# Mesoptier/ray-marching

Hardware: AMD Instinct MI355X
Metric: Mpixels/s at 1920x1080, 256-step march, 32-node SDF (higher is better)
Workload: dtype f32; 1 GPU; 1920x1080, g32 (31 commands / 111 words), 256 max steps, 16 rays/px, RGBA32F out; camera=still, kernel=0, specialized_kernel=True, jit_from_disk_cache=True, frames_in_flight=4

## Files before the change

### ray-marching_amd/csrc/rm_jit.h

```cpp
#pragma once
#include <algorithm>
#include <atomic>
#include <chrono>
#include <condition_variable>
#include <cstdio>
#include <cstdlib>
#include <cstring>
#include <dlfcn.h>
#include <sys/stat.h>
#include <unistd.h>
#include <map>
#include <memory>
#include <mutex>
#include <string>
#include <thread>
#include <vector>

#include "rm_device.h"
#include "rm_units.h"

namespace rmjit {

#include "generated/rm_jit_sources.inc"

// ... 531 lines not shown
            const int w = nv++;
            char an[16], am[16], bn[16], bm[16];
            std::snprintf(an, sizeof an, "v%d", a); std::snprintf(am, sizeof am, "m%d", a);
            std::snprintf(bn, sizeof bn, "v%d", b); std::snprintf(bm, sizeof bm, "m%d", b);
            if (!combine(w, an, am, bn, bm)) return false;
            stack.push_back(w);
            continue;
        }
        const char* fn = kind == RM_KIND_SPHERE ? "sdf_sphere_t<FAST>" : kind == RM_KIND_BOX ? "sdf_box_t<FAST>"
                       : kind == RM_KIND_CYLINDER ? "sdf_cylinder_t<FAST>" : nullptr;
        const int c = pos.back();
        const int leaf = nv++;
        if (fn) std::snprintf(line, sizeof line, "    const float v%d = %s(x%d, y%d, z%d, mp[%u].p, tiny);\n", leaf, fn, c, c, c, r);
        else if (kind == RM_KIND_PLANE)
            std::snprintf(line, sizeof line, "    const float v%d = ((x%d * mp[%u].p[0] + y%d * mp[%u].p[1]) + z%d * mp[%u].p[2]) + mp[%u].p[3];\n", leaf, c, r, c, r, c, r, r);
        else return false;
        s += line;
        if (fn) s += "    guard_fence(tiny);\n";
        if (++leaves % 2 == 0) s += "    __builtin_amdgcn_sched_barrier(0);\n";
        if (mode == RM_MODE_PUSH) {
            std::snprintf(line, sizeof line, "    const uint32_t m%d = 0u;\n", leaf);
            s += line;
            stack.push_back(leaf);
        } else {
            if (stack.empty() || mode == RM_MODE_SMOOTH) return false;
            const int a = stack.back(); stack.pop_back();
            const int w = nv++;
            char an[16], am[16], bn[16];
            std::snprintf(an, sizeof an, "v%d", a); std::snprintf(am, sizeof am, "m%d", a); std::snprintf(bn, sizeof bn, "v%d", leaf);
            if (!combine(w, an, am, bn, "0u")) return false;
            stack.push_back(w);
        }
    }
    if (stack.empty()) return false;
    std::snprintf(line, sizeof line, "    return m%d;\n}\n}  // namespace rmk\n", stack.back());
    s += line;
    *out = std::move(s);
    return true;
}

inline const char* kernel_name() { return "rm_render_v5_spec"; }

inline bool structure_allows_bound_walk(const std::vector<RmRecord>& rec) {
    bool smooth = false;
    int spilled = 0, depth = 0;
    for (const RmRecord& r : rec) {
        const uint32_t kind = RM_OP_KIND(r.op);
        if (kind == RM_KIND_XFORM || kind == RM_KIND_MATERIAL) return false;
        smooth = smooth || RM_OP_MODE(r.op) == RM_MODE_SMOOTH || RM_OP_MODE(r.op) == RM_MODE_INTER || kind == RM_KIND_PLANE;
        if (kind == RM_KIND_POP) spilled--;
        else if (r.op & RM_OP_SPILL) spilled++;
        depth = spilled > depth ? spilled : depth;
    }
    return smooth && depth <= 1;
}

inline bool generate_source(const std::vector<RmRecord>& rec, const std::vector<RmRecord>& mrec, int wpt, int prune_kind, std::string* out,
                            bool* walk_generated = nullptr, bool* taps4_generated = nullptr, std::string* capped_out = nullptr) {
    const bool materials = !mrec.empty();
    const bool with_stats = (prune_kind & KERNEL_WITH_STATS) != 0;
    const bool range_proved = range_variant(prune_kind, materials);
    prune_kind &= PRUNE_KIND_MASK;
    std::string body, taps, walk, unit_walk;
    if (!generate_scene_code(rec, prune_kind, 1, &body, &unit_walk)) return false;
    const bool walk_spec = materials && mrec.size() <= kMaxRecords && generate_material_walk(mrec, &walk);
    if (walk_generated) *walk_generated = walk_spec;
    const bool taps4 = generate_scene_code(rec, prune_kind, 4, &taps);
    if (taps4_generated) *taps4_generated = taps4;
    std::string s;
    s += "typedef unsigned char rm_rtc_u8;\ntypedef unsigned short rm_rtc_u16;\ntypedef unsigned int rm_rtc_u32;\n"
         "typedef unsigned long long rm_rtc_u64;\ntypedef int rm_rtc_i32;\ntypedef long long rm_rtc_i64;\n"
         "#define uint8_t rm_rtc_u8\n#define uint16_t rm_rtc_u16\n#define uint32_t rm_rtc_u32\n#define uint64_t rm_rtc_u64\n"
         "#define int32_t rm_rtc_i32\n#define int64_t rm_rtc_i64\n";
    s += "#define RM_JIT_TU 1\n";
    if (prune_kind == PRUNE_LATTICE) s += "#define RM_JIT_PRUNE_ON 1\n";
    if (prune_kind == PRUNE_BLEND) s += "#define RM_JIT_BLEND_PRUNE 1\n";
    if (taps4) s += "#define RM_JIT_TAPS4 1\n";
    if (walk_spec) s += "#define RM_JIT_MATERIAL_WALK 1\n";
    if (structure_allows_bound_walk(rec)) s += "#define RM_JIT_BOUND_WALK 1\n";
    if (!with_stats) s += "#define RM_NO_WAVE_STATS 1\n";
    if (range_proved) s += "#define RM_JIT_RANGE_PROOF 1\n";
    if (!unit_walk.empty()) s += "#define RM_JIT_UNIT_WALK 1\n";
    if (prune_kind && jit_knob("RM_JIT_PRUNE_STATS", 0) == 5) s += "#define RM_JIT_WALK_COUNTER 1\n";
    s += "#include \"rm_kernel_v5.h\"\n";
    s += body;
    s += unit_walk;
    if (taps4) s += taps;
    if (walk_spec) s += walk;
    char line[512];
    int waves = prune_kind == PRUNE_BLEND ? 6 : 0;
    bool chain = !materials && taps4 && prune_kind != PRUNE_BLEND && !rec.empty();
    for (size_t i = 1; chain && i < rec.size(); i++) {
        const uint32_t kind = RM_OP_KIND(rec[i].op), mode = RM_OP_MODE(rec[i].op);
        chain = (kind == RM_KIND_SPHERE || kind == RM_KIND_BOX || kind == RM_KIND_CYLINDER || kind == RM_KIND_PLANE) && mode != RM_MODE_PUSH;
    }
    if (chain) waves = 7;
    const bool probe = capped_out && waves == 0 && prune_kind == PRUNE_LATTICE && !materials && jit_knob("RM_JIT_PROBE_CAP", 1) != 0;
    auto kernel_text = [&](int w) {
        std::string k;
        if (w > 0) {
            std::snprintf(line, sizeof line, "__attribute__((amdgpu_waves_per_eu(%d, %d)))\n", w, w);
            k += line;
        }
        std::snprintf(line, sizeof line,
                      "extern \"C\" __global__ __launch_bounds__(%d) void %s(RmLaunch L, rmk::V5Work work, uint32_t n_tiles, "
                      "uint32_t refill_min) {\n    rmk::rm_render_v5_body<rmk::ProgLds, true, %d, false, true, %s>(L, work, n_tiles, refill_min);\n}\n",
                      64 * wpt, kernel_name(), wpt, materials ? "true" : "false");
        k += line;
        return k;
    };
    if (capped_out) *capped_out = probe ? s + kernel_text(6) : std::string();
    s += kernel_text(waves);
    *out = std::move(s);
    return true;
}

struct CacheHeader {
    char magic[8];
    uint64_t bytes;
    uint64_t checksum;
    uint64_t reserved;
};
inline uint64_t fnv1a(const char* p, size_t n, uint64_t h = 1469598103934665603ull) {
    for (size_t i = 0; i < n; i++) { h ^= (unsigned char)p[i]; h *= 1099511628211ull; }
    return h;
}
inline const char* const* compile_options(int* n) {
    static const char* const opts[] = {"--offload-arch=gfx950", "-O3", "-std=c++17", "-ffp-contract=off", "-fno-slp-vectorize"};
    *n = (int)(sizeof opts / sizeof *opts);
    return opts;
}
inline std::string cache_dir() {
    if (const char* env = std::getenv("RM_JIT_CACHE_DIR")) return (env[0] == 0 || std::strcmp(env, "off") == 0) ? std::string() : std::string(env);
    Dl_info info;
    std::memset(&info, 0, sizeof info);
    if (!dladdr(reinterpret_cast<void*>(&cache_dir), &info) || !info.dli_fname) return std::string();
    std::string lib(info.dli_fname);
    const size_t slash = lib.rfind('/');
    if (slash == std::string::npos) return std::string();
    return lib.substr(0, slash) + "/jit_cache";
}
inline std::string cache_path(const std::string& src) {
    const std::string dir_s = cache_dir();
    const char* dir = dir_s.empty() ? nullptr : dir_s.c_str();
    Rtc& rtc = Rtc::get();
    if (!dir || !rtc.ok()) return std::string();
    uint64_t h = fnv1a(src.data(), src.size());
    for (int i = 0; i < kNumHeaders; i++) h = fnv1a(kHeaderSources[i], std::strlen(kHeaderSources[i]), h);
    int n_opts = 0;
    const char* const* opts = compile_options(&n_opts);
    for (int i = 0; i < n_opts; i++) h = fnv1a(opts[i], std::strlen(opts[i]) + 1, h);
    h = fnv1a(rtc.identity.data(), rtc.identity.size(), h);
    char name[64];
    std::snprintf(name, sizeof name, "/rm_%016llx.co", (unsigned long long)h);
    return std::string(dir) + name;
}

inline bool compile(const std::string& src, std::vector<char>* code, std::string* log, double* ms, bool* from_cache = nullptr) {
    Rtc& rtc = Rtc::get();
    if (from_cache) *from_cache = false;
    if (!rtc.ok()) { *log = rtc.error; return false; }
    const auto t0 = std::chrono::steady_clock::now();
    const std::string cache_file = cache_path(src);
    if (!cache_file.empty()) {
        if (FILE* f = std::fopen(cache_file.c_str(), "rb")) {
            CacheHeader hd;
// ... 258 lines not shown
```

### ray-marching_amd/csrc/rm_kernel_v5.h

```cpp
#pragma once
#include "rm_interp.h"
#include "rm_lds_layout.h"

namespace rmk {

typedef const __attribute__((address_space(3))) float* LdsF;
RM_DEV LdsF lds_vector_base(const void* generic_lds_ptr) {
    const uint32_t s = (uint32_t)(__SIZE_TYPE__)(const __attribute__((address_space(3))) void*)generic_lds_ptr;
    uint32_t v;
    asm("v_mov_b32 %0, %1" : "=v"(v) : "s"(s));
    return (LdsF)(__SIZE_TYPE__)v;
}
template <bool FAST>
RM_DEV float map_scene_spec(LdsF lp, float qx, float qy, float qz, unsigned long long need, unsigned long long live, SqrtGuard& tiny, uint32_t& n_eval);
#ifdef RM_JIT_UNIT_WALK
template <bool FAST>
RM_DEV float map_scene_walk(LdsF lp, float qx, float qy, float qz, unsigned long long need, unsigned long long live, SqrtGuard& tiny, uint32_t& n_eval);
#define RM_MAP_SCENE_STEP map_scene_walk
#else
#define RM_MAP_SCENE_STEP map_scene_spec
#endif
#ifdef RM_JIT_MATERIAL_WALK
template <bool FAST>
RM_DEV uint32_t map_scene_material_spec(const RmRecord* __restrict__ mp, float qx, float qy, float qz, SqrtGuard& tiny);
// ... 451 lines not shown
                const float slope = CONE ? nd - nn * (rho * 1.00001f) : nd;
                const float away = 1.0e-5f * nn;
                b = slope >= away ? v0 - (1.0e-5f * (__builtin_fabsf(v0) + __builtin_fabsf(p[3])) + nn * (4.0f * lower)) : -inf;
                bounded = false;
            } else if (kind == RM_KIND_SPHERE) {
                const float cx = __builtin_fmaf(my, dz, -(mz * dy)), cy = __builtin_fmaf(mz, dx, -(mx * dz)), cz = __builtin_fmaf(mx, dy, -(my * dx));
                const float perp2 = __builtin_fmaf(cz, cz, __builtin_fmaf(cy, cy, cx * cx));
                reach = fmax_(p[3], 0.0f);
                const float along = __builtin_fmaf(mz, dz, __builtin_fmaf(my, dy, mx * dx));
                const float dist = __builtin_amdgcn_sqrtf(along > 0.0f ? perp2 : mm);
                b = dist * (1.0f - 1.0e-5f) - p[3];
            } else {
                const bool cyl = kind == RM_KIND_CYLINDER;
                const float hx = fmax_(p[3], 0.0f), hy = fmax_(p[4], 0.0f), hz = cyl ? hx : fmax_(p[5], 0.0f);
                reach = (hx + hy) + hz;
                const float x1 = (mx - hx) * ix, x2 = (mx + hx) * ix, y1 = (my - hy) * iy, y2 = (my + hy) * iy;
                const float z1 = (mz - hz) * iz, z2 = (mz + hz) * iz;
                const float nx = fmin_(x1, x2), fx = fmax_(x1, x2), ny = fmin_(y1, y2), fy = fmax_(y1, y2);
                const float nz = fmin_(z1, z2), fz = fmax_(z1, z2);
                const float d0 = fmax_((nx - fy) * wxy, (ny - fx) * wxy);
                const float d1 = fmax_((nx - fz) * wxz, (nz - fx) * wxz);
                const float d2 = fmax_((ny - fz) * wyz, (nz - fy) * wyz);
                const float d3 = fmax_(-fx * ax, fmax_(-fy * ay, -fz * az));
                const float delta = fmax_(fmax_(d0, d1), fmax_(d2, d3));
                b = delta * (1.0f - 1.0e-5f);
            }
            if (CONE && bounded) b = b - (rho * 1.00001f) * ((__builtin_amdgcn_sqrtf(mm) * 1.00001f + reach) + fmax_(b, 0.0f));
            b = fmax_(b - (lower + 1.0e-5f * __builtin_fabsf(b)), -3.0e38f);
            if (op & RM_OP_SPILL) spilled = acc;
            a = acc;
        }
        if (mode == RM_MODE_PUSH) acc = b;
        else if (mode == RM_MODE_UNION) acc = fmin_(a, b);
        else if (mode == RM_MODE_SUB) acc = a;
        else if (mode == RM_MODE_INTER) acc = fmax_(a, b);
        else {
            const float kk = p[0];
            float v = fmin_(a, b);
            if (kk > 0.0f) {
                const float h = fmax_(kk - __builtin_fabsf(a - b), 0.0f) * __builtin_amdgcn_rcpf(kk);
                v = v - ((h * h) * kk) * 0.25f;
                v = v - (1.0e-6f * (__builtin_fabsf(v) + kk));
            }
            acc = fmax_(v, -3.0e38f);
        }
    }
    return acc;
}
template <bool CONE, class LoadRecord>
RM_DEV bool ray_misses_by_bounds_v5(const LoadRecord& load, uint32_t n_rec, const V4& ro, float dx, float dy, float dz, float min_dist,
                                    float scale, float rho = 0.0f) {
    const float acc = ray_bound_v5<CONE>(load, n_rec, ro, dx, dy, dz, scale, rho);
    const float margin = fmax_(min_dist, 0.0f) * 1.01f + 1.0e-4f * scale;
    return acc > margin;
}

struct V5Work {
    const uint32_t* order;
    uint32_t* counters;
    uint32_t* measured;
    const uint32_t* masks;
};

RM_DEV float select_by_mask(float a, float b, unsigned long long m) {
    float r;
    asm("v_cndmask_b32_e64 %0, %1, %2, %3" : "=v"(r) : "v"(a), "v"(b), "s"(m));
    return r;
}
RM_DEV uint32_t select_by_mask(uint32_t a, uint32_t b, unsigned long long m) {
    uint32_t r;
    asm("v_cndmask_b32_e64 %0, %1, %2, %3" : "=v"(r) : "v"(a), "v"(b), "s"(m));
    return r;
}
RM_DEV bool lane_of(unsigned long long m, uint32_t lane) {
    uint32_t r;
    asm("v_cndmask_b32_e64 %0, 0, 1, %1" : "=v"(r) : "s"(m));
    (void)lane;
    return r != 0u;
}

struct TrueTag { static constexpr bool value = true; };
struct FalseTag { static constexpr bool value = false; };

template <class Prog, bool PROG_IN_LDS, int WPT, bool EXT, bool SPEC, bool MAT = false, int LOOP = 0>
RM_DEV void rm_render_v5_body(const RmLaunch& L, const V5Work& work, uint32_t n_tiles, uint32_t refill_min) {
    extern __shared__ __attribute__((aligned(16))) uint32_t smem[];
    const uint32_t tid = threadIdx.x;
    const uint32_t lane = tid & 63u, wave = tid >> 6;
    typedef rml::MarchWaveLds WL;
    float* res = reinterpret_cast<float*>(smem);
    uint32_t* wbase = smem + V5_POOL + wave * L.wave_dwords;
    uint32_t* rq_rid = wbase + WL::rq_rid / 4u;
    float* rq_d = reinterpret_cast<float*>(wbase + WL::rq_d / 4u);
    uint32_t* sq_rid = wbase + WL::sq_rid / 4u;
    float* sq_v = reinterpret_cast<float*>(wbase + WL::sq_v / 4u);
    uint32_t* hq_rid = wbase + WL::hq_rid / 4u;
    float* hq_v = reinterpret_cast<float*>(wbase + WL::hq_v / 4u);
    float* wxy = reinterpret_cast<float*>(wbase + WL::wxy / 4u);
    float* tn = reinterpret_cast<float*>(wbase + WL::tn / 4u);
    uint32_t* after = smem + V5_POOL + WPT * L.wave_dwords;
    float* spill = reinterpret_cast<float*>(after) + wave * (L.spill_depth * 64u) + lane;
    float4* t_cone = reinterpret_cast<float4*>(after + WPT * L.spill_depth * 64u);
    float4* t_slab = t_cone + L.n_cone;
    uint32_t* lprog = reinterpret_cast<uint32_t*>(t_slab + 3u * L.n_slab);
    uint32_t* s_next = lprog + (PROG_IN_LDS ? (L.n_rec + L.n_grp + L.n_tree) * 8u : 0u);
    uint32_t* s_tile = s_next + 1;
    uint32_t* s_veto = s_next + 2;
    float* s_off = reinterpret_cast<float*>(s_next + rml::kMarchCtlBytes / 4u);
    uint8_t* rmat = reinterpret_cast<uint8_t*>(s_next) + rml::kMarchCtlBytes + rml::kMarchOffBytes;
    uint32_t* s_mask = reinterpret_cast<uint32_t*>(rmat + (MAT && L.n_mrec != 0u ? V5_POOL : 0u));
    const bool tagged = MAT && L.n_mrec != 0u;
    constexpr uint32_t TAP_IDLE = MAT ? 5u : 4u;
    const CullTables cullt{t_cone, t_slab, s_veto, L.n_cone, L.n_slab};

    rm_uniforms u = L.u;
    if (L.frames) u = L.frames[blockIdx.z];
    const uint32_t tiles_x = (L.W + 7u) / 8u;
    const uint32_t* order = work.order + (size_t)blockIdx.z * n_tiles;
    uint32_t* counters = work.counters + 4u * blockIdx.z;
    const uint32_t n_active = counters[0];

    const V4 ro = matvec(u.inv_view, 0.0f, 0.0f, 0.0f, 1.0f);
    const float prune_scale = L.scene_scale + ((__builtin_fabsf(ro.x) + __builtin_fabsf(ro.y)) + __builtin_fabsf(ro.z));
    const float thr_c0 = step_thr_c0(prune_scale, ro.x, ro.y, ro.z);
    const float eps = 0.0001f;
    if (PROG_IN_LDS) {
        const uint32_t* src = reinterpret_cast<const uint32_t*>(L.prog);
        for (uint32_t k = tid; k < L.n_rec * 8u; k += 64u * WPT) lprog[SPEC ? ((k & ~7u) | ((k + 7u) & 7u)) : k] = src[k];
        stage_units(lprog + 8u * L.n_rec, L.prog + L.n_rec, L.n_grp, tid, 64u * WPT);
        if constexpr (!SPEC) stage_tree(lprog + 8u * (L.n_rec + L.n_grp), L.prog + L.n_rec + L.n_grp, L.n_tree, tid, 64u * WPT);
    }
    if (tid == 0u) *s_veto = 0u;
    if (tid < 16u) sample_offset(u, tid >> 2, tid & 3u, s_off[2u * tid], s_off[2u * tid + 1u]);
    __syncthreads();
    if (L.flags & 1u)
        for (uint32_t k = tid; k < L.n_rec; k += 64u * WPT) cull_build_v5(L.prog[k], ro, L.min_dist, L.smooth_slack, t_cone, t_slab, s_veto, L.bounds);

    Prog prog;
    if constexpr (PROG_IN_LDS) prog.base = lprog;
    else prog.base = L.prog;

    auto load_record = [&](uint32_t i, uint32_t& op, float (&p)[7]) {
        if constexpr (PROG_IN_LDS) {
            const uint32_t* r = lprog + 8u * i;
            op = r[SPEC ? 7u : 0u];
#pragma unroll
            for (int k = 0; k < 7; k++) p[k] = __uint_as_float(r[(SPEC ? 0u : 1u) + (uint32_t)k]);
        } else {
            prog.load(i, op, p);
        }
    };
    const float bound_scale = prune_scale + L.smooth_slack;
    const LdsF lprog_v = lds_vector_base(lprog);
    uint32_t n_eval = 0u;
    const uint32_t* lunits = lprog + 8u * L.n_rec;
    auto units_needed = [&](float x, float y, float z, float thr, float extra_margin, bool is_live, unsigned long long live_mask) -> unsigned long long {
        if constexpr (SPEC) {
#if defined(RM_JIT_PRUNE_ON)
            return wave_cull_lattice(lunits, L.n_grp, x, y, z, thr, is_live, live_mask);
#elif defined(RM_JIT_BLEND_PRUNE)
            return wave_cull_blend(lunits, L.n_grp, L.unit_kmax, x, y, z, extra_margin, prune_scale, is_live, live_mask);
#else
            return ~0ull;
#endif
        } else if constexpr (LOOP == 2 || LOOP == 4) {
            return wave_cull_lattice(lunits, L.n_grp, x, y, z, thr, is_live, live_mask);
        } else if constexpr (LOOP == 1 || LOOP == 3) {
            return ~0ull;
        } else if constexpr (PROG_IN_LDS) {
            if ((L.flags & 8u) == 0u) return ~0ull;
            if (L.unit_mode == RM_UNITS_LATTICE) return wave_cull_lattice(lunits, L.n_grp, x, y, z, thr, is_live, live_mask);
            return wave_cull_blend(lunits, L.n_grp, L.unit_kmax, x, y, z, extra_margin, prune_scale, is_live, live_mask);
        } else {
            return ~0ull;
        }
    };
    auto eval_scene = [&](float x, float y, float z, float thr, bool is_live, unsigned long long live_mask) -> float {
        float qx[1] = {x}, qy[1] = {y}, qz[1] = {z}, v[1];
        SqrtGuard tiny;
        if constexpr (SPEC) {
            const unsigned long long need = units_needed(x, y, z, thr, 0.0f, is_live, live_mask);
            v[0] = RM_MAP_SCENE_STEP<true>(lprog_v, x, y, z, need, live_mask, tiny, n_eval);
            if (tiny.any_bad()) {
                asm volatile("");
                uint32_t again = 0u;
                v[0] = RM_MAP_SCENE_STEP<false>(lprog_v, x, y, z, need, live_mask, tiny, again);
            }
        } else if (LOOP == 1 || LOOP == 2 || (LOOP == 0 && (L.flags & 4u))) {
            const unsigned long long need = units_needed(x, y, z, thr, 0.0f, is_live, live_mask);
            const bool masked = LOOP == 0 ? (PROG_IN_LDS && (L.flags & 8u) != 0u) : LOOP == 2;
#ifdef RM_INTERP_STATS
            n_eval += (uint32_t)__builtin_popcountll(masked ? need : (L.n_rec >= 64u ? ~0ull : (1ull << L.n_rec) - 1ull));
#endif
            v[0] = map_scene_chain<true>(prog, L.n_rec, x, y, z, need, masked, tiny);
            if (tiny.any_bad()) v[0] = map_scene_chain<false>(prog, L.n_rec, x, y, z, need, masked, tiny);
        } else if (LOOP == 3 || LOOP == 4 || (LOOP == 0 && !EXT)) {
            const bool masked = LOOP == 0 ? (PROG_IN_LDS && (L.flags & 8u) != 0u) : LOOP == 4;
            if (masked) {
                const unsigned long long need = units_needed(x, y, z, thr, 0.0f, is_live, live_mask);
                const TreeKeep k = tree_keep(lunits + 8u * L.n_grp, L.n_rec, need);
#ifdef RM_INTERP_STATS
                n_eval += (uint32_t)(__builtin_popcountll(k.keep0) + __builtin_popcountll(k.keep1));
#endif
                v[0] = map_scene_tree_masked<true>(prog, spill, x, y, z, k.keep0, k.keep1, k.push0, k.push1, tiny);
                if (tiny.any_bad()) v[0] = map_scene_tree_masked<false>(prog, spill, x, y, z, k.keep0, k.keep1, k.push0, k.push1, tiny);
            } else {
                v[0] = map_scene_tree<true>(prog, L.n_rec, spill, x, y, z, tiny);
                if (tiny.any_bad()) v[0] = map_scene_tree<false>(prog, L.n_rec, spill, x, y, z, tiny);
            }
        } else if (PROG_IN_LDS && (L.flags & 8u)) {
            const unsigned long long need = units_needed(x, y, z, thr, 0.0f, is_live, live_mask);
            const uint32_t* ranges = lunits + 7u * L.n_grp;
            v[0] = map_scene_units<true, EXT>(prog, ranges, spill, x, y, z, need, tiny, L.value_spill_depth);
            if (tiny.any_bad())
                v[0] = map_scene_units<false, EXT>(prog, ranges, spill, x, y, z, need, tiny, L.value_spill_depth);
        } else {
            map_scene_multi<1, true, Prog, EXT>(prog, L.n_rec, spill, L.max_dist, qx, qy, qz, v, tiny, L.value_spill_depth);
            if (tiny.any_bad()) map_scene_multi<1, false, Prog, EXT>(prog, L.n_rec, spill, L.max_dist, qx, qy, qz, v, tiny, L.value_spill_depth);
        }
        return v[0];
    };

    enum : uint32_t { START_MARCH = 0u, START_HIT = 1u, START_DONE = 2u };
    const float f0 = __uint_as_float(__builtin_amdgcn_readfirstlane(counters[2]));
    uint32_t start = START_DONE;
    if (L.max_iter != 0u)
        start = f0 < L.min_dist ? START_HIT : (f0 > L.max_dist || L.max_iter <= 1u) ? START_DONE : START_MARCH;
    const float inf_f = __uint_as_float(0x7F800000u);
#if defined(RM_JIT_PRUNE_ON)
    constexpr bool ANCHOR = SPEC;
#elif defined(RM_PRUNE_PLUMBING)
    constexpr bool ANCHOR = !SPEC && (LOOP == 2 || LOOP == 4);
#else
    constexpr bool ANCHOR = false;
#endif
    float anc_x = 0.0f, anc_y = 0.0f, anc_z = 0.0f, anc_t = inf_f;
    unsigned long long anc_due = 0ull;

    const unsigned long long t_start = L.stats ? __builtin_amdgcn_s_memrealtime() : 0ull;
    uint32_t n_iter = 0u, n_live = 0u, n_prod = 0u, n_tiles_done = 0u;

  for (;;) {
    if (tid == 0u) {
        *s_tile = atomicAdd(&counters[1], 1u);
        *s_next = 0u;
        s_next[3] = 0u;
    }
    __syncthreads();
    const uint32_t slot = *s_tile;
    if (slot >= n_active) break;
    const uint32_t tile = order[slot];
    const uint32_t tile_x = tile % tiles_x, tile_y = tile / tiles_x;
    n_tiles_done++;
    const unsigned long long tile_t0 = work.measured ? __builtin_amdgcn_s_memrealtime() : 0ull;

    if (lane < 16u) {
        const uint32_t k = lane & 7u, tx = tile_x * 8u + k, ty = tile_y * 8u + k;
        wxy[lane] = lane < 8u ? screen_x(tx < L.W ? tx : L.W - 1u, L.W)
                              : screen_y(rm_global_row(L, ty < L.rows ? ty : L.rows - 1u), L.H);
    }
    if (lane == 0u) *s_mask = work.masks[(size_t)blockIdx.z * n_tiles + tile];
    __builtin_amdgcn_fence(__ATOMIC_ACQ_REL, "wavefront");

    float dx = 0.f, dy = 0.f, dz = 0.f, sc = 0.f;
    constexpr uint32_t ITR_EMPTY = 0x80000000u, ITR_RETIRED = 0x40000000u;
    uint32_t itr = ITR_EMPTY;
    auto lane_empty = [&]() { return (int32_t)itr < 0; };
    auto lane_marching = [&]() { return itr < ITR_RETIRED; };
    const uint32_t iter_limit = L.max_iter << 10;
    float thr_base = inf_f;
    uint32_t rq_pos = 0u, rq_cnt = 0u, sq_n = 0u, hq_n = 0u;
    uint32_t tap_t = TAP_IDLE, tap_n = 0u;
    bool pool_open = true;

    auto flush_misses = [&]() {
        __builtin_amdgcn_fence(__ATOMIC_ACQ_REL, "wavefront");
        if (lane < sq_n) res[sq_rid[lane]] = miss_code(ro, sq_v[lane], sq_v[V5_SQ + lane], sq_v[2u * V5_SQ + lane]);
        __builtin_amdgcn_fence(__ATOMIC_ACQ_REL, "wavefront");
        sq_n = 0u;
    };

    for (;;) {
        if (tap_t == TAP_IDLE) {
            const unsigned long long want0 = __ballot(lane_empty());
            const unsigned long long live0 = __ballot(lane_marching());
            if (want0 != 0ull && (live0 == 0ull || (uint32_t)__popcll(want0) >= refill_min)) {
                unsigned long long want = want0;
                while (want != 0ull) {
                    if (rq_pos == rq_cnt) {
                        if (!pool_open) {
                            if (lane_empty()) itr = ITR_RETIRED;
                            break;
                        }
                        uint32_t base = 0u;
                        if (lane == 0u) base = atomicAdd(s_next, 64u);
                        base = __builtin_amdgcn_readfirstlane(base);
                        if (base >= V5_POOL) { pool_open = false; continue; }
                        n_prod++;
                        const uint32_t blk = (uint32_t)(0xEDB87421A965FC30ull >> (4u * (base >> 6))) & 15u;
                        uint32_t ln = lane;
                        asm volatile("" : "+v"(ln));
                        const uint32_t bpx = 2u * (blk & 3u) + (ln & 1u), bpy = 2u * (blk >> 2) + ((ln >> 1) & 1u), s = ln >> 2;
                        const uint32_t r = s * 64u + bpy * 8u + bpx;
                        float gx, gy, gz;
                        gen_ray_at<true>(u.inv_proj, u.inv_view, ro, wxy[bpx], wxy[8u + bpy], s_off[2u * s], s_off[2u * s + 1u], gx, gy, gz);
                        const bool finite_d = __builtin_fabsf(gx) < inf_f && __builtin_fabsf(gy) < inf_f && __builtin_fabsf(gz) < inf_f;
                        const bool test_rays = (L.flags & 1u) != 0u && __builtin_amdgcn_readfirstlane(s_next[3]) < 4u;
                        bool culled = L.max_iter == 0u || (start == START_DONE && finite_d) || (test_rays && ray_misses_scene_v5(cullt, __builtin_amdgcn_readfirstlane(*s_mask), gx, gy, gz));
#if !defined(RM_JIT_TU) || defined(RM_JIT_BOUND_WALK)
                        if (test_rays && (L.flags & 32u) && (*s_veto & 1u) == 0u && bound_scale < 1.0e12f && __ballot(!culled) != 0ull)
                            culled = culled || ray_misses_by_bounds_v5<false>(load_record, L.n_rec, ro, gx, gy, gz, L.min_dist, bound_scale);
#endif
                        if (test_rays && base < 256u && __ballot(culled) == 0ull && lane == 0u) atomicAdd(&s_next[3], 1u);
                        if (culled) res[r] = miss_code(ro, gx, gy, gz);
                        const unsigned long long keep = __ballot(!culled);
                        if (!culled) {
                            const uint32_t e = lane_rank(keep);
                            rq_rid[e] = r;
                            rq_d[e] = gx; rq_d[V5_RQ + e] = gy; rq_d[2u * V5_RQ + e] = gz;
                        }
                        rq_pos = 0u;
                        rq_cnt = (uint32_t)__popcll(keep);
                        __builtin_amdgcn_fence(__ATOMIC_ACQ_REL, "wavefront");
                        continue;
                    }
                    const uint32_t avail = rq_cnt - rq_pos, n_want = (uint32_t)__popcll(want);
                    if (lane_empty()) {
                        const uint32_t rank = lane_rank(want);
                        if (rank < avail) {
                            const uint32_t e = rq_pos + rank;
                            const uint32_t rid = rq_rid[e];
                            dx = rq_d[e]; dy = rq_d[V5_RQ + e]; dz = rq_d[2u * V5_RQ + e];
                            const bool finite_d = __builtin_fabsf(dx) < inf_f && __builtin_fabsf(dy) < inf_f && __builtin_fabsf(dz) < inf_f;
                            const bool shared = finite_d && start == START_MARCH;
                            sc = shared ? 0.0f + f0 : 0.0f;
                            itr = rid | (shared ? 1024u : 0u);
                            thr_base = shared ? __builtin_fabsf(f0) * 2.00002f : inf_f;
                            if constexpr (ANCHOR) {
                                if (shared) thr_base = anchor_thr_base(thr_base, ro.x + dx * sc, ro.y + dy * sc, ro.z + dz * sc, anc_x, anc_y, anc_z, anc_t);
                                thr_base = handout_thr_base(thr_base, thr_c0);
                            }
                        }
                    }
                    rq_pos += n_want < avail ? n_want : avail;
                    if constexpr (ANCHOR) anc_due = ~0ull;
                    __builtin_amdgcn_fence(__ATOMIC_ACQ_REL, "wavefront");
                    want = __ballot(lane_empty());
                }
            }
            const bool any_live = __ballot(lane_marching()) != 0ull;
            if (!any_live && __ballot(lane_empty()) != 0ull) continue;
            if (hq_n >= 64u || (!any_live && hq_n != 0u)) {
                tap_n = hq_n < 64u ? hq_n : 64u;
                hq_n -= tap_n;
                __builtin_amdgcn_fence(__ATOMIC_ACQ_REL, "wavefront");
                tap_t = 0u;
            } else if (!any_live) {
                break;
            }
        }
        const bool tapping = tap_t != TAP_IDLE;
        if constexpr (MAT) {
            if (tap_t == 4u) {
                const uint32_t e = hq_n + lane;
                const float hx = hq_v[e], hy = hq_v[V5_HQ + e], hz = hq_v[2u * V5_HQ + e];
#ifdef RM_JIT_MATERIAL_WALK
                SqrtGuard mtiny;
                uint32_t m = map_scene_material_spec<true>(L.mprog, hx, hy, hz, mtiny);
                if (mtiny.any_bad()) m = map_scene_material_spec<false>(L.mprog, hx, hy, hz, mtiny);
#else
                const uint32_t m = map_scene_material(L.mprog, L.n_mrec, spill, L.mat_value_depth, hx, hy, hz);
#endif
                if (lane < tap_n) {
                    const uint32_t r = hq_rid[e] & 1023u;
                    res[r] = shade_hit<true>(tn[lane], tn[64u + lane], tn[128u + lane], hx, hy, hz);
                    rmat[r] = (uint8_t)m;
                }
                tap_t = TAP_IDLE;
                continue;
// ... 58 lines not shown
                is_live = lane_marching();
                if constexpr (ANCHOR) thr = step_thr(thr_base, sc);
                else thr = thr_base + kPruneAbs * (prune_scale + ((__builtin_fabsf(ex) + __builtin_fabsf(ey)) + __builtin_fabsf(ez)));
            }
            const unsigned long long live_m = __builtin_amdgcn_ballot_w64(is_live);
#ifndef RM_NO_WAVE_STATS
            n_iter++;
            n_live += (uint32_t)__popcll(live_m);
#endif
            const float sd = eval_scene(ex, ey, ez, thr, is_live, live_m);

            if (tapping_i) {
                const float vx = __uint_as_float(__float_as_uint(sd) ^ sgx);
                const float vy = __uint_as_float(__float_as_uint(sd) ^ sgy);
                const float vz = __uint_as_float(__float_as_uint(sd) ^ sgz);
                const float nx = tap_t == 0u ? vx : tn[lane] + vx;
                const float ny = tap_t == 0u ? vy : tn[64u + lane] + vy;
                const float nz = tap_t == 0u ? vz : tn[128u + lane] + vz;
                if (++tap_t == 4u && !tagged) {
                    if (is_live) res[hq_rid[he] & 1023u] = shade_hit<true>(nx, ny, nz, hq_v[he], hq_v[V5_HQ + he], hq_v[2u * V5_HQ + he]);
                    tap_t = TAP_IDLE;
                    break;
                }
                tn[lane] = nx; tn[64u + lane] = ny; tn[128u + lane] = nz;
                if (tap_t == 4u) break;
                continue;
            }

            const unsigned long long hit_mask = live_m & __ballot(sd < L.min_dist);
            const unsigned long long on_m = live_m & ~hit_mask;
            const unsigned long long esc_m = on_m & __ballot(sd > L.max_dist);
            const unsigned long long go_m = on_m & ~esc_m;
            sc = select_by_mask(sc, sc + sd, go_m);
            itr = select_by_mask(itr, itr + 1024u, go_m);
#ifdef RM_PRUNE_PLUMBING
            thr_base = select_by_mask(thr_base, ANCHOR ? step_thr_base(sd, thr_c0) : __builtin_fabsf(sd) * 2.00002f, go_m);
#endif
            const unsigned long long miss_mask = esc_m | (go_m & __ballot(itr >= iter_limit));
            const unsigned long long done_m = hit_mask | miss_mask;
            if constexpr (ANCHOR) {
                if ((done_m | anc_due) == 0ull) continue;
                if (anc_due != 0ull) {
                    const int al = (int)__builtin_ctzll(live_m);
                    const float at = anchor_reach(ex, ey, ez, sd, prune_scale);
                    anc_x = __uint_as_float((uint32_t)__builtin_amdgcn_readlane((int)__float_as_uint(ex), al));
                    anc_y = __uint_as_float((uint32_t)__builtin_amdgcn_readlane((int)__float_as_uint(ey), al));
                    anc_z = __uint_as_float((uint32_t)__builtin_amdgcn_readlane((int)__float_as_uint(ez), al));
                    anc_t = __uint_as_float((uint32_t)__builtin_amdgcn_readlane((int)__float_as_uint(at), al));
                    anc_due = 0ull;
                    if (done_m == 0ull) continue;
                }
            }
            if (done_m == 0ull) continue;
            const bool hit = is_live && sd < L.min_dist, miss = lane_of(miss_mask, lane);
            if (hit_mask != 0ull) {
                if (hit) {
                    const uint32_t e = hq_n + lane_rank(hit_mask);
#ifdef RM_PRUNE_PLUMBING
                    hq_rid[e] = (itr & 1023u) | ((__float_as_uint(__builtin_fabsf(sd)) + 1023u) & ~1023u);
#else
                    hq_rid[e] = itr & 1023u;
#endif
                    hq_v[e] = ex; hq_v[V5_HQ + e] = ey; hq_v[2u * V5_HQ + e] = ez;
                    itr = ITR_EMPTY;
                }
                hq_n += (uint32_t)__popcll(hit_mask);
            }
            if (miss_mask != 0ull) {
                const uint32_t n_miss = (uint32_t)__popcll(miss_mask);
                if (sq_n + n_miss > V5_SQ) flush_misses();
                if (miss) {
                    const uint32_t e = sq_n + lane_rank(miss_mask);
                    sq_rid[e] = itr & 1023u;
                    sq_v[e] = dx; sq_v[V5_SQ + e] = dy; sq_v[2u * V5_SQ + e] = dz;
                    itr = ITR_EMPTY;
                }
                sq_n += n_miss;
            }
            n_idle += (uint32_t)__popcll(done_m);
            if ((live_m & ~done_m) == 0ull || n_idle >= refill_min || hq_n >= 64u) break;
        }
    }
    if (sq_n != 0u) flush_misses();
    __syncthreads();

    for (uint32_t p = tid; p < 64u; p += 64u * WPT) {
        const uint32_t px = tile_x * 8u + (p & 7u), py = tile_y * 8u + (p >> 3);
        if (px < L.W && py < L.rows) {
            constexpr bool kGammaLo = MAT || !kRangeProved, kGammaHiAll = kGammaLo;
            auto sum_samples = [&](auto fast_tag, float& tr, float& tg, float& tb, SqrtGuard& guard) {
                constexpr bool FAST = decltype(fast_tag)::value;
                tr = 0.0f; tg = 0.0f; tb = 0.0f;
#pragma unroll 4
                for (uint32_t s = 0; s < 16u; s++) {
                    const float code = res[s * 64u + p];
                    float cr, cg, cb;
                    if (code >= 0.0f) {
                        cr = 0.4f * code; cg = 0.7f * code; cb = 0.1f * code;
                        if constexpr (MAT) {
                            if (tagged) {
                                const float4 al = L.materials[rmat[s * 64u + p]];
                                cr = al.x * code; cg = al.y * code; cb = al.z * code;
                            }
                        }
                    } else if (code > -2.5f) {
                        const float g = 0.2f * (-1.0f - code);
                        cr = 0.1f + g; cg = 0.1f + g; cb = 0.2f + g;
                    } else {
                        cr = 0.0f; cg = 0.0f; cb = 0.0f;
                    }
                    tr += sqrt_sel<FAST, true, kGammaLo, kGammaHiAll>(cr, guard);
                    tg += sqrt_sel<FAST, true, kGammaLo, true>(cg, guard);
                    tb += sqrt_sel<FAST, true, kGammaLo, kGammaHiAll>(cb, guard);
                }
            };
            float tr, tg, tb;
            SqrtGuard gamma_guard;
            sum_samples(TrueTag(), tr, tg, tb, gamma_guard);
            if (gamma_guard.bad()) sum_samples(FalseTag(), tr, tg, tb, gamma_guard);
            store_pixel(L, blockIdx.z, (size_t)py * L.W + px, tr / 16.0f, tg / 16.0f, tb / 16.0f);
        }
    }
    if (work.measured && tid == 0u) {
        const unsigned long long dt = __builtin_amdgcn_s_memrealtime() - tile_t0;
        work.measured[(size_t)blockIdx.z * n_tiles + tile] = dt > 0xFFFFFFFFull ? 0xFFFFFFFFu : (dt == 0ull ? 1u : (uint32_t)dt);
    }
    __syncthreads();
  }
    if (L.stats && lane == 0u) {
        unsigned long long* st = L.stats + 4ull * (((size_t)blockIdx.z * gridDim.x + blockIdx.x) * WPT + wave);
        st[0] = t_start;
        st[1] = __builtin_amdgcn_s_memrealtime();
        st[2] = ((unsigned long long)n_tiles_done << 32) | n_iter;
#ifdef RM_JIT_WALK_COUNTER
        st[3] = ((unsigned long long)n_eval << 32) | n_live;
#else
        st[3] = ((unsigned long long)(n_eval != 0u ? n_eval : n_prod) << 32) | n_live;
#endif
    }
}

template <class Prog, bool PROG_IN_LDS, int WPT, bool EXT>
__global__ __launch_bounds__(64 * WPT) void rm_render_v5(RmLaunch L, V5Work work, uint32_t n_tiles, uint32_t refill_min) {
    rm_render_v5_body<Prog, PROG_IN_LDS, WPT, EXT, false, EXT>(L, work, n_tiles, refill_min);
}
template <int WPT, int LOOP>
__global__ __launch_bounds__(64 * WPT) __attribute__((amdgpu_waves_per_eu(6, 8)))
void rm_render_v5_lean(RmLaunch L, V5Work work, uint32_t n_tiles, uint32_t refill_min) {
    rm_render_v5_body<ProgLds, true, WPT, false, false, false, LOOP>(L, work, n_tiles, refill_min);
}

constexpr uint32_t V5_PRE_TILES = 4u;
constexpr uint32_t V5_PRE_BLOCK = 32u;
static_assert(V5_PRE_BLOCK >= 1u && V5_PRE_BLOCK <= 64u, "one wave classifies the block, lane = tile");

#if !defined(RM_JIT_TU)
RM_DEV bool rect_cone_v5(const float* m_proj, const float* m_view, const V4& ro, const float (&px)[2], const float (&py)[2], const float (&ox)[2],
                         const float (&oy)[2], float noise, float (&cone_out)[4], float (&corner)[4][3]) {
    float cx = 0.0f, cy = 0.0f, cz = 0.0f, ex[4], ey[4], ez[4], inv_hi = 0.0f;
#pragma unroll
    for (uint32_t c = 0; c < 4u; c++) {
        gen_ray_unnormalized_at(m_proj, m_view, ro, px[c & 1u], py[c >> 1], ox[c & 1u], oy[c >> 1], ex[c], ey[c], ez[c]);
        corner[c][0] = ex[c]; corner[c][1] = ey[c]; corner[c][2] = ez[c];
        const float inv = __builtin_amdgcn_rsqf(__builtin_fmaf(ez[c], ez[c], __builtin_fmaf(ey[c], ey[c], ex[c] * ex[c])));
        ex[c] *= inv; ey[c] *= inv; ez[c] *= inv;
        inv_hi = fmax_(inv_hi, inv);
        cx += ex[c]; cy += ey[c]; cz += ez[c];
    }
    unit_dir(cx, cy, cz);
    float rho2 = 0.0f;
#pragma unroll
    for (uint32_t c = 0; c < 4u; c++) {
        const float ax = ex[c] - cx, ay = ey[c] - cy, az = ez[c] - cz;
        rho2 = fmax_(rho2, __builtin_fmaf(az, az, __builtin_fmaf(ay, ay, ax * ax)));
    }
    const float rho = __builtin_fmaf(2.2f * noise, inv_hi, __builtin_sqrtf(rho2) * 1.001f + 2.0e-6f);
    bool cone_ok = rho < 0.05f;
#pragma unroll
    for (uint32_t c = 0; c < 4u; c++) cone_ok = cone_ok && (ex[c] - cx) * (ex[c] - cx) < 1.0f && (ey[c] - cy) * (ey[c] - cy) < 1.0f && (ez[c] - cz) * (ez[c] - cz) < 1.0f;
    cone_out[0] = cx; cone_out[1] = cy; cone_out[2] = cz;
    cone_out[3] = cone_ok ? rho : __uint_as_float(0x7FC00000u);
    return cone_ok;
}
RM_DEV float cone_noise_v5(const rm_uniforms& u, const V4& ro, uint32_t W, uint32_t H) {
    const float bx = (1.0f + 16.0f / (float)W) + 0.75f / __builtin_fabsf(u.viewport_extent[0]);
    const float by = (1.0f + 16.0f / (float)H) + 0.75f / __builtin_fabsf(u.viewport_extent[1]);
    float mag = (__builtin_fabsf(ro.x) + __builtin_fabsf(ro.y)) + __builtin_fabsf(ro.z);
#pragma unroll
    for (int k = 0; k < 4; k++)
        mag += ((__builtin_fabsf(u.inv_view[4 * k]) + __builtin_fabsf(u.inv_view[1 + 4 * k])) + __builtin_fabsf(u.inv_view[2 + 4 * k])) *
               (((__builtin_fabsf(u.inv_proj[k]) * bx + __builtin_fabsf(u.inv_proj[k + 4]) * by) + __builtin_fabsf(u.inv_proj[k + 8])) +
                __builtin_fabsf(u.inv_proj[k + 12]));
    return 1.0e-6f * mag;
}
RM_DEV bool cone_clears_cone_entry_v5(const CullTables& T, const float2* aux, uint32_t k, float cx, float cy, float cz, float rho) {
    const float4 a = T.cone[k];
    const float t = __builtin_fmaf(aux[k].x, rho, __builtin_fmaf(a.z, cz, __builtin_fmaf(a.y, cy, a.x * cx)));
    return t < a.w;
}
RM_DEV bool cone_clears_slab_sphere_v5(const CullTables& T, const float2* aux, uint32_t k, float cx, float cy, float cz, float rho) {
    const float4 c = T.slab[3u * k + 2u];
    const float t = __builtin_fmaf(aux[T.n_cone + k].x, rho, __builtin_fmaf(c.z, cz, __builtin_fmaf(c.y, cy, c.x * cx)));
    return t < c.w;
}
RM_DEV bool cone_clears_slab_box_v5(const CullTables& T, const float2* aux, uint32_t k, float rho, float ix, float iy, float iz) {
    const float infl = aux[T.n_cone + k].y * rho;
    const float4 a = T.slab[3u * k], b = T.slab[3u * k + 1u];
    const float x1 = (a.x - infl) * ix, x2 = (b.x + infl) * ix, y1 = (a.y - infl) * iy, y2 = (b.y + infl) * iy;
    const float z1 = (a.z - infl) * iz, z2 = (b.z + infl) * iz;
    const float tn = fmax_(fmin_(x1, x2), fmax_(fmin_(y1, y2), fmin_(z1, z2)));
    const float tf = fmin_(fmax_(x1, x2), fmin_(fmax_(y1, y2), fmax_(z1, z2)));
    return infl < __uint_as_float(0x7F800000u) && !(tf >= fmax_(tn, 0.0f));
}
RM_DEV bool cone_misses_tables_v5(const CullTables& T, const float2* aux, const float (&cone)[4], bool cone_ok, uint32_t mask) {
    const float cx = cone[0], cy = cone[1], cz = cone[2], rho = cone[3];
    bool clear = cone_ok && *T.veto == 0u;
    if (mask != V5_MASK_ALL) {
        for (uint32_t m = mask_cone_bits(mask, T.n_cone); m != 0u; m &= m - 1u)
// ... 550 lines not shown
```

Measured before the change: 7853 Mpixels/s.

## Claim next tile during resolve and spread sample resolve across all waves

The next tile's slot, tile index and mask are now claimed by a second wave while the resolve phase runs, rather than in a separate atomic-plus-barrier step at the top of each tile loop. This hides the global atomic and mask load behind the resolve work. For specialized kernels with at least four waves, the gamma/sqrt work for the 16 samples is split across the waves, each writing partial roots into its LDS region. Wave 0 then sums them, so the resolve no longer runs on one wave alone. This adds a barrier and LDS traffic, and it reuses the wave scratch region. An optional timer for the handover gap is also added behind a stats knob.

```diff
diff --git a/ray-marching_amd/csrc/rm_jit.h b/ray-marching_amd/csrc/rm_jit.h
--- a/ray-marching_amd/csrc/rm_jit.h
+++ b/ray-marching_amd/csrc/rm_jit.h
@@ -637,6 +637,7 @@
     if (range_proved) s += "#define RM_JIT_RANGE_PROOF 1\n";
     if (!unit_walk.empty()) s += "#define RM_JIT_UNIT_WALK 1\n";
     if (prune_kind && jit_knob("RM_JIT_PRUNE_STATS", 0) == 5) s += "#define RM_JIT_WALK_COUNTER 1\n";
+    if (with_stats && jit_knob("RM_JIT_PRUNE_STATS", 0) == 6) s += "#define RM_JIT_HANDOVER_TIMER 1\n";
     s += "#include \"rm_kernel_v5.h\"\n";
     s += body;
     s += unit_walk;
diff --git a/ray-marching_amd/csrc/rm_kernel_v5.h b/ray-marching_amd/csrc/rm_kernel_v5.h
--- a/ray-marching_amd/csrc/rm_kernel_v5.h
+++ b/ray-marching_amd/csrc/rm_kernel_v5.h
@@ -557,6 +557,9 @@
 struct TrueTag { static constexpr bool value = true; };
 struct FalseTag { static constexpr bool value = false; };
 
+constexpr bool kClaimInResolve = true;
+constexpr bool kWideResolve = true;
+
 template <class Prog, bool PROG_IN_LDS, int WPT, bool EXT, bool SPEC, bool MAT = false, int LOOP = 0>
 RM_DEV void rm_render_v5_body(const RmLaunch& L, const V5Work& work, uint32_t n_tiles, uint32_t refill_min) {
     extern __shared__ __attribute__((aligned(16))) uint32_t smem[];
@@ -584,6 +587,7 @@
     float* s_off = reinterpret_cast<float*>(s_next + rml::kMarchCtlBytes / 4u);
     uint8_t* rmat = reinterpret_cast<uint8_t*>(s_next) + rml::kMarchCtlBytes + rml::kMarchOffBytes;
     uint32_t* s_mask = reinterpret_cast<uint32_t*>(rmat + (MAT && L.n_mrec != 0u ? V5_POOL : 0u));
+    constexpr uint32_t kNoTile = 0xFFFFFFFFu;
     const bool tagged = MAT && L.n_mrec != 0u;
     constexpr uint32_t TAP_IDLE = MAT ? 5u : 4u;
     const CullTables cullt{t_cone, t_slab, s_veto, L.n_cone, L.n_slab};
@@ -605,7 +609,22 @@
         stage_units(lprog + 8u * L.n_rec, L.prog + L.n_rec, L.n_grp, tid, 64u * WPT);
         if constexpr (!SPEC) stage_tree(lprog + 8u * (L.n_rec + L.n_grp), L.prog + L.n_rec + L.n_grp, L.n_tree, tid, 64u * WPT);
     }
-    if (tid == 0u) *s_veto = 0u;
+    auto open_next_tile = [&]() {
+        const uint32_t slot = atomicAdd(&counters[1], 1u);
+        uint32_t tile = kNoTile, mask = 0u;
+        if (slot < n_active) {
+            tile = order[slot];
+            mask = work.masks[(size_t)blockIdx.z * n_tiles + tile];
+        }
+        *s_tile = tile;
+        *s_mask = mask;
+        *s_next = 0u;
+        s_next[3] = 0u;
+    };
+    if (tid == 0u) {
+        *s_veto = 0u;
+        if constexpr (kClaimInResolve) open_next_tile();
+    }
     if (tid < 16u) sample_offset(u, tid >> 2, tid & 3u, s_off[2u * tid], s_off[2u * tid + 1u]);
     __syncthreads();
     if (L.flags & 1u)
@@ -715,16 +734,28 @@
     const unsigned long long t_start = L.stats ? __builtin_amdgcn_s_memrealtime() : 0ull;
     uint32_t n_iter = 0u, n_live = 0u, n_prod = 0u, n_tiles_done = 0u;
 
+#ifdef RM_JIT_HANDOVER_TIMER
+    unsigned long long ho_t0 = 0ull;
+    uint32_t ho_ticks = 0u;
+#endif
+
+    if constexpr (kClaimInResolve) __syncthreads();
   for (;;) {
-    if (tid == 0u) {
-        *s_tile = atomicAdd(&counters[1], 1u);
-        *s_next = 0u;
-        s_next[3] = 0u;
-    }
-    __syncthreads();
-    const uint32_t slot = *s_tile;
-    if (slot >= n_active) break;
-    const uint32_t tile = order[slot];
+    uint32_t tile;
+    if constexpr (kClaimInResolve) {
+        tile = __builtin_amdgcn_readfirstlane(*s_tile);
+        if (tile == kNoTile) break;
+    } else {
+        if (tid == 0u) {
+            *s_tile = atomicAdd(&counters[1], 1u);
+            *s_next = 0u;
+            s_next[3] = 0u;
+        }
+        __syncthreads();
+        const uint32_t slot = *s_tile;
+        if (slot >= n_active) break;
+        tile = order[slot];
+    }
     const uint32_t tile_x = tile % tiles_x, tile_y = tile / tiles_x;
     n_tiles_done++;
     const unsigned long long tile_t0 = work.measured ? __builtin_amdgcn_s_memrealtime() : 0ull;
@@ -734,7 +765,9 @@
         wxy[lane] = lane < 8u ? screen_x(tx < L.W ? tx : L.W - 1u, L.W)
                               : screen_y(rm_global_row(L, ty < L.rows ? ty : L.rows - 1u), L.H);
     }
-    if (lane == 0u) *s_mask = work.masks[(size_t)blockIdx.z * n_tiles + tile];
+    if constexpr (!kClaimInResolve) {
+        if (lane == 0u) *s_mask = work.masks[(size_t)blockIdx.z * n_tiles + tile];
+    }
     __builtin_amdgcn_fence(__ATOMIC_ACQ_REL, "wavefront");
 
     float dx = 0.f, dy = 0.f, dz = 0.f, sc = 0.f;
@@ -770,6 +803,12 @@
                         uint32_t base = 0u;
                         if (lane == 0u) base = atomicAdd(s_next, 64u);
                         base = __builtin_amdgcn_readfirstlane(base);
+#ifdef RM_JIT_HANDOVER_TIMER
+                        if (ho_t0 != 0ull) {
+                            ho_ticks += (uint32_t)(__builtin_amdgcn_s_memrealtime() - ho_t0);
+                            ho_t0 = 0ull;
+                        }
+#endif
                         if (base >= V5_POOL) { pool_open = false; continue; }
                         n_prod++;
                         const uint32_t blk = (uint32_t)(0xEDB87421A965FC30ull >> (4u * (base >> 6))) & 15u;
@@ -994,44 +1033,95 @@
         }
     }
     if (sq_n != 0u) flush_misses();
+#ifdef RM_JIT_HANDOVER_TIMER
+    ho_t0 = __builtin_amdgcn_s_memrealtime();
+#endif
     __syncthreads();
 
-    for (uint32_t p = tid; p < 64u; p += 64u * WPT) {
-        const uint32_t px = tile_x * 8u + (p & 7u), py = tile_y * 8u + (p >> 3);
-        if (px < L.W && py < L.rows) {
-            constexpr bool kGammaLo = MAT || !kRangeProved, kGammaHiAll = kGammaLo;
-            auto sum_samples = [&](auto fast_tag, float& tr, float& tg, float& tb, SqrtGuard& guard) {
-                constexpr bool FAST = decltype(fast_tag)::value;
-                tr = 0.0f; tg = 0.0f; tb = 0.0f;
-#pragma unroll 4
-                for (uint32_t s = 0; s < 16u; s++) {
-                    const float code = res[s * 64u + p];
-                    float cr, cg, cb;
-                    if (code >= 0.0f) {
-                        cr = 0.4f * code; cg = 0.7f * code; cb = 0.1f * code;
-                        if constexpr (MAT) {
-                            if (tagged) {
-                                const float4 al = L.materials[rmat[s * 64u + p]];
-                                cr = al.x * code; cg = al.y * code; cb = al.z * code;
-                            }
-                        }
-                    } else if (code > -2.5f) {
-                        const float g = 0.2f * (-1.0f - code);
-                        cr = 0.1f + g; cg = 0.1f + g; cb = 0.2f + g;
-                    } else {
-                        cr = 0.0f; cg = 0.0f; cb = 0.0f;
-                    }
-                    tr += sqrt_sel<FAST, true, kGammaLo, kGammaHiAll>(cr, guard);
-                    tg += sqrt_sel<FAST, true, kGammaLo, true>(cg, guard);
-                    tb += sqrt_sel<FAST, true, kGammaLo, kGammaHiAll>(cb, guard);
+    constexpr bool kGammaLo = MAT || !kRangeProved, kGammaHiAll = kGammaLo;
+    auto sample_roots = [&](auto fast_tag, uint32_t s, uint32_t p, float& rr, float& rg, float& rb, SqrtGuard& guard) {
+        constexpr bool FAST = decltype(fast_tag)::value;
+        const float code = res[s * 64u + p];
+        float cr, cg, cb;
+        if (code >= 0.0f) {
+            cr = 0.4f * code; cg = 0.7f * code; cb = 0.1f * code;
+            if constexpr (MAT) {
+                if (tagged) {
+                    const float4 al = L.materials[rmat[s * 64u + p]];
+                    cr = al.x * code; cg = al.y * code; cb = al.z * code;
+                }
+            }
+        } else if (code > -2.5f) {
+            const float g = 0.2f * (-1.0f - code);
+            cr = 0.1f + g; cg = 0.1f + g; cb = 0.2f + g;
+        } else {
+            cr = 0.0f; cg = 0.0f; cb = 0.0f;
+        }
+        rr = sqrt_sel<FAST, true, kGammaLo, kGammaHiAll>(cr, guard);
+        rg = sqrt_sel<FAST, true, kGammaLo, true>(cg, guard);
+        rb = sqrt_sel<FAST, true, kGammaLo, kGammaHiAll>(cb, guard);
+    };
+    if constexpr (kWideResolve && SPEC && WPT >= 4) {
+        constexpr uint32_t S = 16u / (uint32_t)WPT;
+        static_assert(WPT <= 16 && S * 3u * 256u <= WL::wxy, "the roots of a wave's samples lie in front of its wxy");
+        const uint32_t px = tile_x * 8u + (lane & 7u), py = tile_y * 8u + (lane >> 3);
+        const bool inside = px < L.W && py < L.rows;
+        float* roots = reinterpret_cast<float*>(wbase);
+        if (inside) {
+            auto wave_roots = [&](auto fast_tag, SqrtGuard& guard) {
+#pragma unroll
+                for (uint32_t k = 0; k < S; k++) {
+                    float rr, rg, rb;
+                    sample_roots(fast_tag, wave * S + k, lane, rr, rg, rb, guard);
+                    roots[(3u * k) * 64u + lane] = rr;
+                    roots[(3u * k + 1u) * 64u + lane] = rg;
+                    roots[(3u * k + 2u) * 64u + lane] = rb;
                 }
             };
-            float tr, tg, tb;
             SqrtGuard gamma_guard;
-            sum_samples(TrueTag(), tr, tg, tb, gamma_guard);
-            if (gamma_guard.bad()) sum_samples(FalseTag(), tr, tg, tb, gamma_guard);
+            wave_roots(TrueTag(), gamma_guard);
+            if (gamma_guard.bad()) wave_roots(FalseTag(), gamma_guard);
+        }
+        __syncthreads();
+        if (wave == 0u && inside) {
+            float tr = 0.0f, tg = 0.0f, tb = 0.0f;
+            const float* r = reinterpret_cast<const float*>(smem + V5_POOL) + lane;
+#pragma unroll 1
+            for (uint32_t w = 0; w < (uint32_t)WPT; w++, r += L.wave_dwords) {
+#pragma unroll
+                for (uint32_t k = 0; k < S; k++) {
+                    tr += r[(3u * k) * 64u];
+                    tg += r[(3u * k + 1u) * 64u];
+                    tb += r[(3u * k + 2u) * 64u];
+                }
+            }
             store_pixel(L, blockIdx.z, (size_t)py * L.W + px, tr / 16.0f, tg / 16.0f, tb / 16.0f);
         }
+    } else {
+        for (uint32_t p = tid; p < 64u; p += 64u * WPT) {
+            const uint32_t px = tile_x * 8u + (p & 7u), py = tile_y * 8u + (p >> 3);
+            if (px < L.W && py < L.rows) {
+                auto sum_samples = [&](auto fast_tag, float& tr, float& tg, float& tb, SqrtGuard& guard) {
+                    tr = 0.0f; tg = 0.0f; tb = 0.0f;
+#pragma unroll 4
+                    for (uint32_t s = 0; s < 16u; s++) {
+                        float rr, rg, rb;
+                        sample_roots(fast_tag, s, p, rr, rg, rb, guard);
+                        tr += rr;
+                        tg += rg;
+                        tb += rb;
+                    }
+                };
+                float tr, tg, tb;
+                SqrtGuard gamma_guard;
+                sum_samples(TrueTag(), tr, tg, tb, gamma_guard);
+                if (gamma_guard.bad()) sum_samples(FalseTag(), tr, tg, tb, gamma_guard);
+                store_pixel(L, blockIdx.z, (size_t)py * L.W + px, tr / 16.0f, tg / 16.0f, tb / 16.0f);
+            }
+        }
+    }
+    if constexpr (kClaimInResolve) {
+        if (tid == (WPT > 1 ? 64u : 0u)) open_next_tile();
     }
     if (work.measured && tid == 0u) {
         const unsigned long long dt = __builtin_amdgcn_s_memrealtime() - tile_t0;
@@ -1046,6 +1136,8 @@
         st[2] = ((unsigned long long)n_tiles_done << 32) | n_iter;
 #ifdef RM_JIT_WALK_COUNTER
         st[3] = ((unsigned long long)n_eval << 32) | n_live;
+#elif defined(RM_JIT_HANDOVER_TIMER)
+        st[3] = ((unsigned long long)ho_ticks << 32) | n_live;
 #else
         st[3] = ((unsigned long long)(n_eval != 0u ? n_eval : n_prod) << 32) | n_live;
 #endif
```

New measurement: 7357 Mpixels/s. 0.937x the previous value.
